# ac-93/tactile_gym

Measured on AMD Instinct MI355X. Metric: env-steps/sec (128x128 tactile obs) at N envs, higher is better.
Workload: dtype f64

## Files before the change

### tactile_gym_amd/csrc/tg_api.hip

```cpp
#include "tg_ctx.hpp"

namespace tg {

int report_error(int code, const char* msg) { return fail(code, msg ? msg : ""); }
static void h_quat_from_euler(const double* rpy, double* q) {
    const double phi = 0.5 * rpy[0], the = 0.5 * rpy[1], psi = 0.5 * rpy[2];
    q[0] = sin(phi) * cos(the) * cos(psi) - cos(phi) * sin(the) * sin(psi);
    q[1] = cos(phi) * sin(the) * cos(psi) + sin(phi) * cos(the) * sin(psi);
    q[2] = cos(phi) * cos(the) * sin(psi) - sin(phi) * sin(the) * cos(psi);
    q[3] = cos(phi) * cos(the) * cos(psi) + sin(phi) * sin(the) * sin(psi);
    const double nrm = sqrt(q[0] * q[0] + q[1] * q[1] + q[2] * q[2] + q[3] * q[3]);
    for (int k = 0; k < 4; ++k) q[k] /= nrm;
}
static void h_mat_from_quat(const double* q, double* R) {
    const double x = q[0], y = q[1], z = q[2], w = q[3];
    const double d = x * x + y * y + z * z + w * w, s = 2.0 / d;
    const double xs = x * s, ys = y * s, zs = z * s, wx = w * xs, wy = w * ys, wz = w * zs, xx = x * xs, xy = x * ys, xz = x * zs, yy = y * ys,
                 yz = y * zs, zz = z * zs;
    R[0] = 1.0 - (yy + zz); R[1] = xy - wz; R[2] = xz + wy;
    R[3] = xy + wz; R[4] = 1.0 - (xx + zz); R[5] = yz - wx;
    R[6] = xz - wy; R[7] = yz + wx; R[8] = 1.0 - (xx + yy);
}


// ... 227 lines not shown
        __syncthreads();
    }
    if (threadIdx.x == 0 && hi[0] > lo[0] && lo[0] != ~0ull) { acc[0] += hi[0] - lo[0]; acc[1] += 1ull; }
}

struct Timer {
    tg_ctx* c; int which; hipEvent_t a = nullptr, b = nullptr;
    Timer(tg_ctx* ctx, int w) : c(ctx), which(w) {
        if ((c->profile || c->profile_clock) && c->d_kt && which < 5) { c->st.kt = c->d_kt; c->rp.kt = c->d_kt; }
        if (c->profile) { (void)hipEventCreate(&a); (void)hipEventCreate(&b); (void)hipEventRecord(a, c->stream); }
    }
    ~Timer() {
        if (c->profile) { (void)hipEventRecord(b, c->stream); c->events.push_back({a, b, which}); }
        if ((c->profile || c->profile_clock) && c->d_kt && which < 5) {
            hipLaunchKernelGGL(k_kt_reduce, dim3(1), dim3(1024), 0, c->stream, c->d_kt, c->kt_slots, c->d_kt_acc + 2 * which);
            c->st.kt = nullptr; c->rp.kt = nullptr;
        }
    }
};


template <typename T, int TOPO> static bool launch_step_t(tg_ctx* c, const float* d_actions, int reset_phase = -1) {
    const int n = c->cfg.num_envs;
    if (c->cfg.control_mode == TG_CONTROL_TCP_POSITION) {
        hipLaunchKernelGGL((k_step_pos<T, TOPO>), dim3((n + 63) / 64), dim3(64), 0, c->stream, (const DevRobot<T>*)c->d_robot,
                           (const EnvConst<T>*)c->d_const, c->st, d_actions);
        return false;
    }
    if constexpr (TOPO == 0 && std::is_same<T, double>::value) {
        if (reset_phase >= 0) {
            hipLaunchKernelGGL((k_step<T, TOPO, true>), dim3((n + 63) / 64), dim3(64), 0, c->stream, (const DevRobot<T>*)c->d_robot,
                               (const EnvConst<T>*)c->d_const, c->st, d_actions, reset_phase, c->bank_mode != 0 ? (const BankDev*)c->d_bank : (const BankDev*)nullptr);
            return true;
        }
    }
    hipLaunchKernelGGL((k_step<T, TOPO>), dim3((n + 63) / 64), dim3(64), 0, c->stream, (const DevRobot<T>*)c->d_robot,
                       (const EnvConst<T>*)c->d_const, c->st, d_actions, -1, (const BankDev*)nullptr);
    return false;
}
template <typename T, int TOPO> static void launch_reset_t(tg_ctx* c, const uint8_t* d_mask, int phase, bool bank = false) {
    const int n = c->cfg.num_envs;
    hipLaunchKernelGGL((k_reset<T, TOPO>), dim3((n + 63) / 64), dim3(64), 0, c->stream, (const DevRobot<T>*)c->d_robot,
                       (const EnvConst<T>*)c->d_const, c->st, d_mask, phase, bank ? (const BankDev*)c->d_bank : (const BankDev*)nullptr);
    if (c->st.kt) c->st.kt += 2 * (size_t)((n + 63) / 64);
}
template <typename T, int TOPO> static void launch_bank_refill_t(tg_ctx* c, int phase) {
    const int n = c->cfg.num_envs;
    hipLaunchKernelGGL((k_bank_refill<T, TOPO>), dim3((n + 63) / 64), dim3(64), 0, c->bank_stream, (const DevRobot<T>*)c->d_robot,
                       (const EnvConst<T>*)c->d_const, c->st, c->bk, c->aux, phase);
}

template <typename T> static void launch_step_body_t(tg_ctx* c, const float* d_actions) {
// ... 587 lines not shown
    if (has_feature) {
        c->packed_feature_off = (c->packed_bytes + 3) & ~(size_t)3;
        c->packed_bytes = c->packed_feature_off + (size_t)n * 12 * 4;
    }
    TG_HIP(hipMalloc(&c->d_obs, c->packed_bytes)); TG_HIP(hipMemset(c->d_obs, 0, c->packed_bytes));
    s.reward = (float*)(c->d_obs + c->packed_obs_bytes);
    s.done = c->d_obs + c->packed_obs_bytes + (size_t)n * 4;
    if (has_feature) s.feature = (float*)(c->d_obs + c->packed_feature_off);
    TG_HIP(hipMalloc(&c->d_term, npix * n)); TG_HIP(hipMemset(c->d_term, 0, npix * n));
    TG_HIP(hipMalloc(&c->d_episode, (size_t)n * 16)); TG_HIP(hipMemset(c->d_episode, 0, (size_t)n * 16));
    s.ep_return = (double*)c->d_episode;
    s.ep_final_return = (float*)(c->d_episode + (size_t)n * 8);
    s.ep_final_len = (int32_t*)(c->d_episode + (size_t)n * 12);
    TG_HIP(hipMalloc(&c->d_mask, n));
#ifdef TG_TL_STAMPS
    TG_HIP(hipMalloc(&s.tl, (4 * 8192 + 4) * 8)); TG_HIP(hipMemset(s.tl, 0, (4 * 8192 + 4) * 8));
#endif
    TG_HIP(hipMalloc(&c->d_actions, (size_t)n * 6 * sizeof(float)));
    c->rp = make_raster_params(W, H, sensor->fov_deg, sensor->near_plane, sensor->far_plane, sensor->turn_off_border, sensor->nodef_dep);
    if (make_block_tables(c->rp, sensor->nodef_dep, sensor->nodef_gray, sensor->border_mask, n, &c->d_block_tables)) return fail(-2, "hipMalloc failed (raster block tables)");
    c->fused_pref = cfg->fused_step == TG_FUSED_OFF ? -1 : cfg->fused_step == TG_FUSED_ON ? 1 : 0;
    if (const char* e = getenv("TG_FUSED_STEP")) c->fused_pref = e[0] == '0' ? -1 : 1;
    c->no_inline_reset = getenv("TG_NO_INLINE_RESET") != nullptr;
#ifdef TG_TL_STAMPS
    c->rp.tl = s.tl;
#endif
    c->bk = s;
    {
        int want = cfg->reset_bank == TG_BANK_OFF ? 0 : cfg->reset_bank == TG_BANK_SYNC ? 2 : 1;
        if (const char* e = getenv("TG_RESET_BANK")) want = (e[0] == '0') ? 0 : (e[0] == 's') ? 2 : 1;
        if (const char* e = getenv("TG_RESET_BANK_EVERY")) { const int k = atoi(e); if (k >= 1) c->bank_every = k; }
        const bool kind_ok = cfg->env_kind == TG_ENV_EDGE_FOLLOW || cfg->env_kind == TG_ENV_SURFACE_FOLLOW_AUTO;
        if (want && kind_ok && cfg->auto_reset && !use_arm_wave(c)) {
            State& b = c->bk;
            auto grab = [&](auto*& ptr, size_t bytes) -> int {
                void* p_ = nullptr;
                if (hipMalloc(&p_, bytes) != hipSuccess) return -1;
                (void)hipMemset(p_, 0, bytes);
                c->bank_allocs.push_back(p_);
                ptr = reinterpret_cast<std::remove_reference_t<decltype(ptr)>>(p_);
                return 0;
            };
            int bad = 0;
            bad |= grab(b.q, nd * 8); bad |= grab(b.qd, nd * 8); bad |= grab(b.qd_target, nd * 8);
            bad |= grab(b.tcp_pos, (size_t)3 * n * 8); bad |= grab(b.tcp_rpy, (size_t)3 * n * 8);
            bad |= grab(b.edge_ang, (size_t)n * 8); bad |= grab(b.embed, (size_t)n * 8); bad |= grab(b.edge_sc, (size_t)2 * n * 8);
// ... 598 lines not shown
```

### tactile_gym_amd/csrc/tg_api_state.hip

```cpp
#include "tg_ctx.hpp"

namespace tg {
template <typename T, int TOPO> static void launch_refresh_t(tg_ctx* c) {
    const int n = c->cfg.num_envs;
    hipLaunchKernelGGL((k_refresh<T, TOPO>), dim3((n + 63) / 64), dim3(64), 0, c->stream, (const DevRobot<T>*)c->d_robot,
                       (const EnvConst<T>*)c->d_const, c->st);
}

template <typename T, int TOPO> static void launch_refresh_rpy_t(tg_ctx* c) {
    const int n = c->cfg.num_envs;
    hipLaunchKernelGGL((k_refresh_rpy<T, TOPO>), dim3((n + 63) / 64), dim3(64), 0, c->stream, (const DevRobot<T>*)c->d_robot,
                       (const EnvConst<T>*)c->d_const, c->st);
}
__global__ __launch_bounds__(256) void k_gather_live_surface(int n, int cells, const uint8_t* __restrict__ hsel, const double* __restrict__ heights,
                                                             const float* __restrict__ zoff, double* __restrict__ out_h, float* __restrict__ out_z) {
    const int env = blockIdx.x;
    const size_t idx = (size_t)(hsel[env] & 3) * n + env;
    if (out_h != nullptr) for (int k = threadIdx.x; k < cells; k += 256) out_h[(size_t)env * cells + k] = heights[idx * cells + k];
    if (out_z != nullptr && threadIdx.x == 0) out_z[env] = zoff[idx];
}
__global__ __launch_bounds__(256) void k_pack_done_rows(const uint8_t* __restrict__ done, const uint8_t* __restrict__ term, const float* __restrict__ ep_ret,
                                                        const int32_t* __restrict__ ep_len, int n, int cap, size_t img, uint8_t* __restrict__ dst) {
    __shared__ int part[256];
    const int env = blockIdx.x, t = threadIdx.x;
// ... 84 lines not shown
    if (!c) return fail(-1, "NULL argument");
    if (!c->d_bp) return fail(-1, "tg_check_broadphase: no guard (tg_set_broadphase)");
    TG_ENTER(c);
    if (launch_broadphase(c->cfg.physics_dtype, c->robot.topology, c->cfg.num_envs, c->stream, c->d_robot, c->d_bp, c->st, c->d_bp_out, c->d_bp_tot))
        return fail(-3, "tg_check_broadphase: unsupported topology");
    TG_HIP(hipGetLastError());
    return 0;
}
int tg_get_broadphase_totals(tg_ctx* c, int64_t* checks, int64_t* pairs, int64_t* hits) {
    if (!c || !checks || !pairs || !hits) return fail(-1, "NULL argument");
    *checks = *pairs = *hits = 0;
    if (!c->d_bp_tot) return 0;
    TG_ENTER(c);
    unsigned long long t[3];
    TG_HIP(hipMemcpyAsync(t, c->d_bp_tot, sizeof t, hipMemcpyDeviceToHost, c->stream));
    TG_HIP(hipStreamSynchronize(c->stream));
    *checks = (int64_t)t[0]; *pairs = (int64_t)t[1]; *hits = (int64_t)t[2];
    return 0;
}

int tg_get_step_mode(tg_ctx* c, int32_t* mode, int32_t* envs_per_wavefront) {
    if (!c || !mode) return fail(-1, "NULL argument");
    *mode = use_fused_step(c) ? 1 : 0;
    if (envs_per_wavefront) *envs_per_wavefront = *mode ? fused_envs_per_wave(c->cfg.num_envs) : 0;
    return 0;
}

int tg_get_actions(tg_ctx* c, void** dev_actions) {
    if (!c || !dev_actions) return fail(-1, "NULL argument");
    *dev_actions = c->d_actions;
    return 0;
}

int tg_get_interior_count(tg_ctx* c, int32_t* k) {
    if (!c || !k) return fail(-1, "NULL argument");
    *k = c->cfg_turn_off_border ? -1 : 4 * c->n_interior;
    return 0;
}
int tg_get_bank_stats(tg_ctx* c, int64_t* swapped, int64_t* late, int32_t* mode) {
    if (!c || !swapped || !late || !mode) return fail(-1, "NULL argument");
    TG_ENTER(c);
    *swapped = 0; *late = 0; *mode = c->bank_mode;
    if (c->st.tmpl_stats != nullptr) {
        unsigned long long t[2] = {0, 0};
        TG_HIP(hipMemcpyAsync(t, c->st.tmpl_stats, 16, hipMemcpyDeviceToHost, c->stream));
        TG_HIP(hipStreamSynchronize(c->stream));
        *swapped = (int64_t)t[0]; *late = (int64_t)t[1]; *mode = c->st.reset_tmpl != nullptr ? 3 : 0;
// ... 177 lines not shown
```

### tactile_gym_amd/csrc/tg_ctx.hpp

```cpp
#pragma once
#include <hip/hip_runtime.h>

#include <chrono>
#include <cmath>
#include <cstdio>
#include <cstdlib>
#include <cstring>
#include <algorithm>
#include <map>
#include <string>
#include <tuple>
#include <type_traits>
#include <vector>

#include "../../include/tactile_gym_hip.h"
#include "tg_kernels.hpp"
#include "tg_contact_wave.h"
#include "tg_spin.h"
#include "tg_fused.h"
#include "tg_scene.h"
#include "tg_noise.h"
#include "tg_raster.h"
#include "tg_exchange.h"
#include "tg_broadphase.h"
// ... 197 lines not shown
    uint64_t random_seed = 0;
    tg::State bk{};
    tg::BankAux aux{};
    int bank_mode = 0;
    uint8_t* h_rows = nullptr;
    size_t h_rows_bytes = 0;
    int bank_every = 8;
    static constexpr int kBankRing = 16, kBankLag = 8;
    hipEvent_t ev_bank_ring[kBankRing] = {};
    unsigned long long bank_visits = 0;
    long long bank_steps = 0;
    hipStream_t bank_stream = nullptr;
    hipEvent_t ev_bank = nullptr, ev_bank_done = nullptr;
    std::vector<void*> bank_allocs;
    void* d_bank = nullptr;
    bool profile = false;
    bool profile_clock = false;
    struct Ev { hipEvent_t a, b; int which; };
    std::vector<Ev> events;
    double prof_ms[6] = {0, 0, 0, 0, 0, 0};
    int64_t prof_n[6] = {0, 0, 0, 0, 0, 0};
    int fused_pref = 0;
    bool no_inline_reset = false;
    unsigned long long* d_kt = nullptr;
    unsigned long long* d_kt_acc = nullptr;
    size_t kt_slots = 0;
    double wall_clock_khz = 100000.0;
};

static inline bool env_has_feature(int env_kind) {
    return env_kind == TG_ENV_OBJECT_PUSH || env_kind == TG_ENV_OBJECT_ROLL || env_kind == TG_ENV_SURFACE_FOLLOW_AUTO;
}

namespace tg {
static void drain_events(tg_ctx* c) {
    for (auto& e : c->events) {
        (void)hipEventSynchronize(e.b);
        float ms = 0;
        (void)hipEventElapsedTime(&ms, e.a, e.b);
        c->prof_ms[e.which] += ms;
        c->prof_n[e.which] += 1;
        (void)hipEventDestroy(e.a); (void)hipEventDestroy(e.b);
    }
    c->events.clear();
}
#define TG_DISPATCH(ctx_dtype, ctx_topo, CALL)                                               \
// ... 54 lines not shown
```

### tactile_gym_amd/csrc/tg_kernels.hpp

```cpp
#pragma once
#include <hip/hip_runtime.h>

#include <stdint.h>

#include "../../include/tactile_gym_hip.h"
#include "tg_physics.hpp"
#include "tg_kt.hpp"

namespace tg {

template <typename T> struct EnvConst {
    int num_envs, act_dim, movement_mode, noise_mode, reward_mode, max_steps, action_repeat, solver_iters;
    T dt, min_action, max_action, act_lo[6], act_hi[6], tcp_lims[6][2];
    T work_pos[3];
    Q4<T> work_q, work_qinv;
    M3<T> work_R, work_Rinv;
    T work_inv_pos[3];
    T stim_pos[3], edge_height, edge_len, term_dist, embed_default;
    double embed_lo, embed_hi;
    M3<T> cam_rot;
    T cam_pos[3];
    int env_kind, surf_rows, surf_cols, surf_goal, surf_vertical;
    M3<T> stim_R;
    double surf_scale, surf_range, surf_interp, surf_extent, auto_scale;
// ... 115 lines not shown
        const double edge = (k == n - 1) ? hi : prod + lo;
        count += (k < n && edge <= v) ? 1 : 0;
    }
    return count;
}
__device__ inline double linspace_value(double lo, double hi, int n, int k) {
#pragma clang fp contract(off)
    const double step = (hi - lo) / (double)(n - 1);
    const double prod = (double)k * step;
    return (k == n - 1) ? hi : prod + lo;
}
__device__ inline double grad_axis(const double* f, int idx, int n, int stride, double h) {
    if (idx == 0) return (f[stride] - f[0]) / h;
    if (idx == n - 1) return (f[(size_t)(n - 1) * stride] - f[(size_t)(n - 2) * stride]) / h;
    return (f[(size_t)(idx + 1) * stride] - f[(size_t)(idx - 1) * stride]) / (2.0 * h);
}

#ifdef TG_KSTEP_STAMPS
__device__ unsigned long long g_kstep_stamps[16];
#define TG_KSTAMP(i) { if (blockIdx.x == 0 && threadIdx.x == 0) g_kstep_stamps[i] = __builtin_readcyclecounter(); asm volatile("" ::: "memory"); }
#else
#define TG_KSTAMP(i)
#endif
__device__ __forceinline__ void episode_step(const State& st, int env, float reward, bool done, int step_count) {
    const double acc = st.ep_return[env] + (double)reward;
    if (done) { st.ep_final_return[env] = (float)acc; st.ep_final_len[env] = step_count; }
    st.ep_return[env] = done ? 0.0 : acc;
}

template <typename T, int TOPO>
__device__ __forceinline__ bool finish_env(const DevRobot<T>& m, const EnvConst<T>& c, const State& st, int env, const T (&q)[Topo<TOPO>::N],
                                           T edge_ang, int step_count, bool write_reward_done, const JointTrig<T, Topo<TOPO>::N>* trig = nullptr,
                                           bool lazy_rpy = false ) {
    const int n = c.num_envs;
    bool done_flag = false;
    Kin<T, TOPO> k;
    if (trig != nullptr) forward_kinematics<T, TOPO, true>(m, q, k, trig);
    else forward_kinematics<T, TOPO>(m, q, k);
    V3<T> ptcp; M3<T> Rtcp;
    link_frame<T, TOPO>(k, m.tcp_link, m.tcp_pos, m.tcp_rot, ptcp, Rtcp);
    st.tcp_pos[0 * n + env] = (double)ptcp.x; st.tcp_pos[1 * n + env] = (double)ptcp.y; st.tcp_pos[2 * n + env] = (double)ptcp.z;
    if (!lazy_rpy) {
        T rpy[3];
        { Q4<T> qq = quat_from_mat(Rtcp); euler_from_quat(qq, rpy[0], rpy[1], rpy[2]); }
        st.tcp_rpy[0 * n + env] = (double)rpy[0]; st.tcp_rpy[1 * n + env] = (double)rpy[1]; st.tcp_rpy[2 * n + env] = (double)rpy[2];
    }
    T se = T(0), ce = T(1);
    if (c.env_kind == TG_ENV_EDGE_FOLLOW) {
        if (lazy_rpy) { se = (T)st.edge_sc[0 * n + env]; ce = (T)st.edge_sc[1 * n + env]; }
        else { tsincos(edge_ang, &se, &ce); st.edge_sc[0 * n + env] = (double)se; st.edge_sc[1 * n + env] = (double)ce; }
    }
    if (write_reward_done && c.env_kind == TG_ENV_EDGE_FOLLOW) {
        const T gx = c.stim_pos[0] + c.edge_len * ce, gy = c.stim_pos[1] + c.edge_len * se;
        const T dx = ptcp.x - gx, dy = ptcp.y - gy;
        const T goal_dist = tsqrt(dx * dx + dy * dy);
        const bool done = goal_dist < c.term_dist || step_count >= c.max_steps;
        const T p1x = c.stim_pos[0] - c.edge_len * ce, p1y = c.stim_pos[1] - c.edge_len * se;
        const T d21x = gx - p1x, d21y = gy - p1y, d13x = p1x - ptcp.x, d13y = p1y - ptcp.y;
        const T edge_dist = tabs(d21x * d13y - d21y * d13x) / tsqrt(d21x * d21x + d21y * d21y);
        T reward;
        if (c.reward_mode == TG_REWARD_SPARSE) reward = goal_dist < c.term_dist ? T(1) : T(0);
        else reward = -((T(1) * goal_dist) + (T(10) * edge_dist) + T(0));
        st.reward[env] = (float)reward;
        st.done[env] = done ? 1 : 0;
        done_flag = done;
        episode_step(st, env, (float)reward, done, step_count);
    }
    TG_KSTAMP(5)
    if ((write_reward_done || c.reward_mode == TG_REWARD_SPARSE) && c.env_kind == TG_ENV_SURFACE_FOLLOW_AUTO) {
        const int R = c.surf_rows, Cc = c.surf_cols;
        int ti = digitize_linspace((double)ptcp.y, c.ybin_lo, c.ybin_hi, Cc);
        int tj = digitize_linspace((double)ptcp.x, c.xbin_lo, c.xbin_hi, R);
        if (ti == Cc) ti -= 1;
        if (tj == R) tj -= 1;
        const double* H = st.heights + ((size_t)(st.hsel[env] & 3) * n + env) * R * Cc;
        const T surf_z = (T)(H[(size_t)ti * Cc + tj] + (double)c.stim_pos[2]);
        const T gy_ = (T)grad_axis(H + tj, ti, R, Cc, c.surf_scale);
        const T gx_ = (T)grad_axis(H + (size_t)ti * Cc, tj, Cc, 1, c.surf_scale);
        V3<T> nrm{-gx_, -gy_, T(1)};
        nrm = (T(1) / norm(nrm)) * nrm;
        const T gdx = ptcp.x - (T)st.goal[0 * n + env], gdy = ptcp.y - (T)st.goal[1 * n + env], gdz = ptcp.z - (T)st.goal[2 * n + env];
        T reward;
        if (c.surf_vertical) {
            nrm = mul(c.stim_R, nrm);
            const V3<T> tipv = mul(Rtcp, mk(T(-1), T(0), T(0)));
            const V3<T> emb = mul(Rtcp, mk(-c.embed_default, T(0), T(0)));
            const T surf_x = (T)((double)c.stim_pos[0] - H[(size_t)ti * Cc + tj]);
            const T surf_dist = tabs((ptcp.x + emb.x) - surf_x);
            const T cos_sim = dot(nrm, tipv) / (norm(nrm) * norm(tipv));
            reward = -((T(10) * surf_dist) + (T(3) * (T(1) - cos_sim)));
        } else {
            const V3<T> tipv = mul(Rtcp, mk(T(0), T(0), T(-1)));
            const V3<T> emb = mul(Rtcp, mk(T(0), T(0), -c.embed_default));
            const T surf_dist = tabs((ptcp.z + emb.z) - surf_z);
            const T cos_sim = dot(nrm, tipv) / (norm(nrm) * norm(tipv));
            const T w_norm = (c.movement_mode == TG_SMOVE_YZ || c.movement_mode == TG_SMOVE_XYZ) ? T(0) : T(1);
            reward = c.surf_goal ? -((T(1) * tsqrt(gdx * gdx + gdy * gdy)) + (T(10) * surf_dist) + (w_norm * (T(1) - cos_sim)))
                                 : -((T(1) * surf_dist) + (w_norm * (T(1) - cos_sim)));
        }
        const bool at_goal = tsqrt(gdx * gdx + gdy * gdy + gdz * gdz) < c.term_dist;
        T out = reward;
        if (c.reward_mode == TG_REWARD_SPARSE) {
            const double acc = st.accum[env] + (double)reward;
            st.accum[env] = acc;
            out = at_goal ? (T)acc : T(0);
        }
        if (write_reward_done) {
            st.reward[env] = (float)out;
            st.done[env] = (at_goal || step_count >= c.max_steps) ? 1 : 0;
            done_flag = at_goal || step_count >= c.max_steps;
            episode_step(st, env, (float)out, at_goal || step_count >= c.max_steps, step_count);
        }
    }
    if (c.env_kind == TG_ENV_SURFACE_FOLLOW_AUTO && st.feature != nullptr) {
        const V3<T> tw_ = load_v3(c.work_inv_pos) + mul(c.work_Rinv, ptcp);
        const V3<T> gw_ = load_v3(c.work_inv_pos) + mul(c.work_Rinv, mk((T)st.goal[0 * n + env], (T)st.goal[1 * n + env], (T)st.goal[2 * n + env]));
        const float f[6] = {(float)tw_.x, (float)tw_.y, (float)tw_.z, (float)gw_.x, (float)gw_.y, (float)gw_.z};
#pragma unroll
        for (int e = 0; e < 6; ++e) {
            st.feature[(size_t)env * 12 + e] = f[e];
            if (write_reward_done) st.term_feature[(size_t)env * 12 + e] = f[e];
        }
    }
    TG_KSTAMP(6)
    V3<T> pb; M3<T> Rb;
    link_frame<T, TOPO>(k, m.sensor_link, m.sensor_pos, m.sensor_rot, pb, Rb);
    const V3<T> pc = pb + mul(Rb, load_v3(c.cam_pos));
    const M3<T> Rc = mul(Rb, c.cam_rot);
    V3<T> f{Rc.m[0], Rc.m[3], Rc.m[6]}, up{Rc.m[2], Rc.m[5], Rc.m[8]};
    f = (T(1) / norm(f)) * f;
    V3<T> s = cross(f, up);
    s = (T(1) / norm(s)) * s;
    const V3<T> u = cross(s, f);
    V3<T> ox{ce, se, T(0)}, oy{-se, ce, T(0)}, oz{T(0), T(0), T(1)};
    if (c.surf_vertical) {
        ox = mk(c.stim_R.m[0], c.stim_R.m[3], c.stim_R.m[6]); oy = mk(c.stim_R.m[1], c.stim_R.m[4], c.stim_R.m[7]);
        oz = mk(c.stim_R.m[2], c.stim_R.m[5], c.stim_R.m[8]);
    }
    const V3<T> dp = load_v3(c.stim_pos) - pc;
    const V3<T> nf = mk<T>(0, 0, 0) - f;
    float* X = st.stim_xform;
    X[0 * n + env] = (float)dot(s, ox);  X[1 * n + env] = (float)dot(s, oy);  X[2 * n + env] = (float)dot(s, oz);
    X[3 * n + env] = (float)dot(u, ox);  X[4 * n + env] = (float)dot(u, oy);  X[5 * n + env] = (float)dot(u, oz);
    X[6 * n + env] = (float)dot(nf, ox); X[7 * n + env] = (float)dot(nf, oy); X[8 * n + env] = (float)dot(nf, oz);
    X[9 * n + env] = (float)dot(s, dp);  X[10 * n + env] = (float)dot(u, dp); X[11 * n + env] = (float)dot(nf, dp);
    return done_flag;
}

template <typename T, int TOPO>
__global__ __launch_bounds__(64) void k_oracle_obs(const DevRobot<T>* __restrict__ mp, const EnvConst<T>* __restrict__ cp, State st, int dim,
                                                   float* __restrict__ out) {
    constexpr int N = Topo<TOPO>::N;
// ... 158 lines not shown
            for (int r = 0; r < 3; ++r) g[r] = (double)c.work_pos[r] + ((double)c.work_R.m[3 * r + 0] * wx + (double)c.work_R.m[3 * r + 1] * wy);
            put_sphere(i, g, 0.01f, i < gid ? 255.0f : 0.0f, i > gid ? 255.0f : 0.0f, i == gid ? 255.0f : 0.0f);
        }
    } else if (c.env_kind == TG_ENV_OBJECT_ROLL) {
        const M3<T> Rq = mat_from_quat(quat_from_mat(Rtcp));
        const V3<T> gw = ptcp + mul(Rq, mk((T)st.goal[0 * n + env], (T)st.goal[1 * n + env], (T)st.goal[2 * n + env]));
        const double g[3] = {(double)gw.x, (double)gw.y, (double)gw.z};
        put_sphere(0, g, 0.0025f, 255.0f, 0.0f, 0.0f);
    } else {
        for (int i = 0; i < n_spheres; ++i) S[8 * i + 7] = 0.0f;
    }
}

template <typename T> __device__ __forceinline__ void scale_actions(const EnvConst<T>& c, const T (&enc)[6], T (&vels)[6]) {
    const T in_range = c.max_action - c.min_action;
#pragma unroll
    for (int d = 0; d < 6; ++d) {
        T x = enc[d];
        x = x < c.min_action ? c.min_action : (x > c.max_action ? c.max_action : x);
        vels[d] = (((x - c.min_action) * (c.act_hi[d] - c.act_lo[d])) / in_range) + c.act_lo[d];
    }
}

template <typename T, int TOPO>
__device__ __forceinline__ void tcp_velocity_control(const DevRobot<T>& m, const EnvConst<T>& c, const T (&q)[Topo<TOPO>::N], T (&vels)[6],
                                                     T (&qd_des)[Topo<TOPO>::N], const JointTrig<T, Topo<TOPO>::N>* trig = nullptr,
                                                     T work_dz = T(0) ) {
    constexpr int N = Topo<TOPO>::N;
    Kin<T, TOPO> k;
    if (trig != nullptr) forward_kinematics<T, TOPO, true>(m, q, k, trig);
    else forward_kinematics<T, TOPO>(m, q, k);
    V3<T> ptcp; M3<T> Rtcp;
    link_frame<T, TOPO>(k, m.tcp_link, m.tcp_pos, m.tcp_rot, ptcp, Rtcp);
    TG_KSTAMP(10)
    V3<T> wpos; T wrpy[3] = {T(0), T(0), T(0)}, rpyw[3];
    if (__any(vels[3] != T(0) || vels[4] != T(0) || vels[5] != T(0)))
        world_to_work<T, false>(c, mk(ptcp.x, ptcp.y, ptcp.z - work_dz), Rtcp, wpos, wrpy, rpyw);
    else
        wpos = load_v3(c.work_inv_pos) + mul(c.work_Rinv, mk(ptcp.x, ptcp.y, ptcp.z - work_dz));
    const T cur[6] = {wpos.x, wpos.y, wpos.z, wrpy[0], wrpy[1], wrpy[2]};
#pragma unroll
    for (int d = 0; d < 6; ++d) {
        const bool ex = (cur[d] < c.tcp_lims[d][0] && vels[d] < T(0)) || (cur[d] > c.tcp_lims[d][1] && vels[d] > T(0));
        if (ex) vels[d] = T(0);
    }
    const V3<T> lin = mul(c.work_R, mk(vels[0], vels[1], vels[2]));
    const V3<T> ang = mul(c.work_R, mk(vels[3], vels[4], vels[5]));
    TG_KSTAMP(11)
    T J[6][N];
    tcp_jacobian<T, TOPO>(m, k, ptcp, J);
    TG_KSTAMP(12)
    if (N == 6) {
        T A[6][6], b[6] = {lin.x, lin.y, lin.z, ang.x, ang.y, ang.z}, x[6];
#pragma unroll
        for (int r = 0; r < 6; ++r)
#pragma unroll
            for (int cc = 0; cc < 6; ++cc) A[r][cc] = J[r][cc < N ? cc : 0];
        solve_pivoted<T, 6>(A, b, x);
#pragma unroll
        for (int i = 0; i < N; ++i) qd_des[i] = x[i < 6 ? i : 0];
    } else {
        const T b[6] = {lin.x, lin.y, lin.z, ang.x, ang.y, ang.z};
        pinv_apply<T, N>(J, b, qd_des);
        if (N == 8) { qd_des[N - 3] = qd_des[1]; qd_des[N - 2] = -qd_des[1]; qd_des[N - 1] = qd_des[1] + qd_des[2]; }
    }
}

template <typename T>
__device__ __forceinline__ void encode_arm_actions(const EnvConst<T>& c, const State& st, int env, const float* __restrict__ a, T (&enc)[6]) {
    const int n = c.num_envs;
    if (c.env_kind == TG_ENV_EDGE_FOLLOW) {
        enc[0] = (T)a[0]; enc[1] = (T)a[1];
        if (c.movement_mode == TG_MOVE_XYZ) enc[2] = (T)a[2];
        else if (c.movement_mode == TG_MOVE_XYRZ) enc[5] = (T)a[2];
        else if (c.movement_mode == TG_MOVE_XYZRZ) { enc[2] = (T)a[2]; enc[5] = (T)a[3]; }
    } else if (c.surf_goal) {
        if (c.movement_mode == TG_SMOVE_YZ) { enc[1] = (T)a[0]; enc[2] = (T)a[1]; }
        else if (c.movement_mode == TG_SMOVE_YZRX) { enc[1] = (T)a[0]; enc[2] = (T)a[1]; enc[3] = (T)a[2]; }
        else {
            enc[0] = (T)a[0]; enc[1] = (T)a[1]; enc[2] = (T)a[2];
            if (c.movement_mode == TG_SMOVE_XYZRXRY) { enc[3] = (T)a[3]; enc[4] = (T)a[4]; }
        }
    } else if (c.surf_vertical) {
        enc[1] = (T)((st.dir[1 * n + env] * (double)c.max_action) * c.auto_scale);
        enc[0] = (T)a[0]; enc[5] = (T)a[1];
    } else {
        enc[0] = (T)((st.dir[0 * n + env] * (double)c.max_action) * c.auto_scale);
        enc[1] = (T)((st.dir[1 * n + env] * (double)c.max_action) * c.auto_scale);
        enc[2] = (T)a[0];
        if (c.movement_mode == TG_SMOVE_YZRX) enc[3] = (T)a[1];
        else if (c.movement_mode == TG_SMOVE_XYZRXRY) { enc[3] = (T)a[1]; enc[4] = (T)a[2]; }
    }
}

template <typename T, int TOPO>
__device__ __forceinline__ bool step_env(const DevRobot<T>& m, const EnvConst<T>& c, const State& st, int env, const float* __restrict__ actions,
                                         bool* done_out = nullptr ) {
    constexpr int N = Topo<TOPO>::N;
    const int n = c.num_envs;
    TG_KSTAMP(0)
    T q[N], qd[N];
#pragma unroll
    for (int i = 0; i < N; ++i) { q[i] = (T)st.q[i * n + env]; qd[i] = (T)st.qd[i * n + env]; }
    T enc[6] = {T(0), T(0), T(0), T(0), T(0), T(0)};
    if (st.draw != nullptr) {
        const uint64_t counter = st.draw[0] + 1, seed = st.draw[1];
        const float lo = (float)c.min_action, hi = (float)c.max_action;
        float abuf[6] = {0.0f, 0.0f, 0.0f, 0.0f, 0.0f, 0.0f};
#pragma unroll
        for (int j = 0; j < 6; ++j) {
            if (j < c.act_dim) {
                const int i = env * c.act_dim + j;
                const uint64_t z = mix64(mix64(seed + kGolden * (counter + 1)) + kGolden * (uint64_t)(i + 1));
                const float u = (float)(uint32_t)(z >> 40) * (1.0f / 16777216.0f);
                abuf[j] = lo + (hi - lo) * u;
                st.act_out[i] = abuf[j];
            }
        }
        encode_arm_actions<T>(c, st, env, abuf, enc);
    } else {
        encode_arm_actions<T>(c, st, env, actions + (size_t)env * c.act_dim, enc);
    }
    T vels[6];
    scale_actions<T>(c, enc, vels);
    const int step_count = st.step_count[env] + 1;
    st.step_count[env] = step_count;
    JointTrig<T, N> trig;
    const int lic = st.licence[env];
    if (__all(lic > 0)) {
#pragma unroll
        for (int i = 0; i < N; ++i) { trig.s[i] = (T)st.trig_sc[i * n + env]; trig.c[i] = (T)st.trig_sc[(8 + i) * n + env]; }
    } else {
        trig_init<T, N>(q, trig);
    }
    T qd_des[N];
    TG_KSTAMP(1)
    tcp_velocity_control<T, TOPO>(m, c, q, vels, qd_des, &trig);
    TG_KSTAMP(2)
#pragma unroll
    for (int i = 0; i < N; ++i) st.qd_target[i * n + env] = (double)qd_des[i];

    T qdummy[N];
#pragma unroll
    for (int i = 0; i < N; ++i) qdummy[i] = T(0);
    int verified = __all(lic > 0) ? 24 : 0;
    bool ran_full = false;
    int sweeps = 0;
    for (int t = 0; t < c.action_repeat; ++t) {
        const int before = verified;
        sim_tick<T, TOPO, kMotorVelocity, true, true>(m, q, qd, qdummy, qd_des, T(0), m.vel_gain, m.max_force, c.dt, c.solver_iters, &trig,
                                                      &verified, &sweeps);
        const bool analytic = before > 0 && verified == before - 1;
        if (t == 0) TG_KSTAMP(7)
        if (!analytic) ran_full = true;
        if (verified < 0) verified = 0;
        const int remaining = c.action_repeat - t - 1;
        if (analytic && remaining > 0 && verified >= remaining && c.solver_iters >= 0) {
            T v2 = T(0);
#pragma unroll
            for (int i = 0; i < N; ++i) v2 += qd[i] * qd[i];
// ... 4 lines not shown
                for (int i = 0; i < N; ++i) dq[i] = c.dt * qd[i];
                for (int r = 0; r < remaining; ++r) {
#pragma unroll
                    for (int i = 0; i < N; ++i) q[i] += dq[i];
                }
                T dqt[N];
#pragma unroll
                for (int i = 0; i < N; ++i) dqt[i] = (T)remaining * dq[i];
                trig_advance<T, N>(q, dqt, trig);
                verified -= remaining;
                break;
            }
        }
    }
    st.licence[env] = ran_full ? (verified > 0 ? 8 : 0) : lic - 1;
    if (m.res_thr > T(0)) st.sweeps[env] = sweeps;
    TG_KSTAMP(3)

#pragma unroll
    for (int i = 0; i < N; ++i) { st.q[i * n + env] = (double)q[i]; st.qd[i * n + env] = (double)qd[i]; }
#pragma unroll
    for (int i = 0; i < N; ++i) { st.trig_sc[i * n + env] = (double)trig.s[i]; st.trig_sc[(8 + i) * n + env] = (double)trig.c[i]; }
    TG_KSTAMP(4)
    const bool done = finish_env<T, TOPO>(m, c, st, env, q, (T)st.edge_ang[env], step_count, true, &trig, true);
    if (done_out != nullptr) *done_out = done;
    return ran_full;
}
constexpr int kDrawGroups = 32, kDrawWords = 16 + 16 * kDrawGroups;
__device__ __forceinline__ void draw_counter_advance(const State& st) {
    if (st.draw != nullptr) {
        __syncthreads();
        if (threadIdx.x == 0) {
            bool last = true;
            if (gridDim.x > 2 * kDrawGroups) {
                const unsigned g = blockIdx.x % kDrawGroups;
                const unsigned long long members = (gridDim.x - g + kDrawGroups - 1) / kDrawGroups;
                unsigned long long* tk = st.draw + 16 + 16 * g;
                last = atomicAdd(tk, 1ull) == members - 1;
                if (last) { atomicExch(tk, 0ull); last = atomicAdd(st.draw + 2, 1ull) == (unsigned long long)kDrawGroups - 1; }
            } else {
                last = atomicAdd(st.draw + 2, 1ull) == (unsigned long long)gridDim.x - 1;
            }
            if (last) { atomicExch(st.draw + 2, 0ull); atomicAdd(st.draw + 0, 1ull); }
        }
    }
}

// ... 7 lines not shown
        const unsigned g = blockIdx.x % kDrawGroups;
        const unsigned long long members = (gridDim.x - g + kDrawGroups - 1) / kDrawGroups;
        last = ticket == members - 1;
        if (last) { atomicExch(st.draw + 16 + 16 * g, 0ull); last = atomicAdd(st.draw + 2, 1ull) == (unsigned long long)kDrawGroups - 1; }
    } else {
        last = ticket == (unsigned long long)gridDim.x - 1;
    }
    if (last) { atomicExch(st.draw + 2, 0ull); atomicAdd(st.draw + 0, 1ull); }
}

template <typename T, int TOPO> __device__ __forceinline__ void reset_or_swap(const DevRobot<T>* __restrict__ mp, const EnvConst<T>* __restrict__ cp, const State& st,
                                                                             int env, bool in_step, int phase, const BankDev* __restrict__ bd);
template <typename T, int TOPO, bool RESET = false>
__global__ __launch_bounds__(64) void k_step(const DevRobot<T>* __restrict__ mp, const EnvConst<T>* __restrict__ cp, State st,
                                             const float* __restrict__ actions, int reset_phase, const BankDev* __restrict__ bd) {
    KtScope kt_scope_(st.kt);
    const int env = blockIdx.x * blockDim.x + threadIdx.x;
    TG_TL(st.tl, 1);
    if (env >= cp->num_envs) return;
    bool done = false;
    const bool ran_full = step_env<T, TOPO>(*mp, *cp, st, env, actions, &done);
    if (RESET) {
        if (done) reset_or_swap<T, TOPO>(mp, cp, st, env, true, reset_phase, bd);
    }
    draw_counter_advance(st);
    TG_KSTAMP(9)
#ifdef TG_KSTEP_STAMPS
    if (blockIdx.x == 0 && threadIdx.x == 0) g_kstep_stamps[15] = ran_full ? 1 : 0;
#else
    (void)ran_full;
#endif
}

template <typename T> __device__ __forceinline__ V3<T> rot_error(const M3<T>& Rt, const M3<T>& R) {
    M3<T> E;
#pragma unroll
    for (int i = 0; i < 3; ++i)
#pragma unroll
        for (int j = 0; j < 3; ++j) E.m[3 * i + j] = Rt.m[3 * i] * R.m[3 * j] + Rt.m[3 * i + 1] * R.m[3 * j + 1] + Rt.m[3 * i + 2] * R.m[3 * j + 2];
    const T cosang = T(0.5) * (E.m[0] + E.m[4] + E.m[8] - T(1));
    const V3<T> ax{E.m[7] - E.m[5], E.m[2] - E.m[6], E.m[3] - E.m[1]};
    const T s = norm(ax);
    const T ang = tatan2(T(0.5) * s, cosang);
    if (s < T(1e-12)) return T(0.5) * ax;
    return (ang / s) * ax;
}
// ... 1330 lines not shown
```

### tactile_gym_amd/csrc/tg_physics.hpp

```cpp
#pragma once
#include <hip/hip_runtime.h>
#include <stdint.h>

#include <type_traits>

namespace tg {

constexpr int kMaxDof = 8;
constexpr int kMaxBodiesPerLink = 4;

template <int TOPO> struct Topo;
template <> struct Topo<0> {
    static constexpr int N = 6;
    static constexpr int NP = 6;
    __host__ __device__ static constexpr int parent(int i) { return i - 1; }
};
template <> struct Topo<1> {
    static constexpr int N = 8;
    static constexpr int NP = 5;
    __host__ __device__ static constexpr int parent(int i) { return i == 0 ? -1 : (i == 5 ? 0 : i - 1); }
};
template <int TOPO> __host__ __device__ constexpr bool is_ancestor_or_self(int anc, int i) {
    while (i >= 0) { if (i == anc) return true; i = Topo<TOPO>::parent(i); }
    return false;
// ... 169 lines not shown
        if (p < 0) {
            k.R[i] = Rl;
            k.o[i] = load_v3(m.jpos[i]);
        } else {
            k.R[i] = mul(k.R[p], Rl);
            k.o[i] = k.o[p] + mul(k.R[p], load_v3(m.jpos[i]));
        }
        k.a[i] = mul(k.R[i], ax);
    }
}

template <typename T, int TOPO> __device__ __forceinline__ void link_frame(const Kin<T, TOPO>& k, int link, const T* fpos, const T* frot,
                                                                             V3<T>& pos, M3<T>& rot) {
    constexpr int N = Topo<TOPO>::N;
#pragma unroll
    for (int i = 0; i < N; ++i) {
        if (i == link) {
            pos = k.o[i] + mul(k.R[i], load_v3(fpos));
            rot = mul(k.R[i], load_m3(frot));
        }
    }
}

template <typename T, int TOPO, bool BIAS = true, bool TRIG = false>
__device__ __forceinline__ void dynamics_terms(const DevRobot<T>& m, const T (&q)[Topo<TOPO>::N], const T (&qd)[Topo<TOPO>::N],
                                               T (&hbias)[Topo<TOPO>::N], T (&qdamp)[Topo<TOPO>::N],
                                               T (&Minv)[Topo<TOPO>::N][Topo<TOPO>::N], T& traceM, const V3<T> g, Kin<T, TOPO>& k,
                                               const JointTrig<T, Topo<TOPO>::N>* trig = nullptr) {
    constexpr int N = Topo<TOPO>::N;
    forward_kinematics<T, TOPO, TRIG>(m, q, k, trig);
    V3<T> w[N], wd[N], vo[N], ao[N];
    V3<T> WF[N], WN[N], DF[N], DN[N], hc[N];
    S3<T> Io[N];
    T mc[N];
#pragma unroll
    for (int i = 0; i < N; ++i) {
        const int p = Topo<TOPO>::parent(i);
        const V3<T> aq = qd[i] * k.a[i];
        if (p < 0) {
            w[i] = aq;
            vo[i] = mk<T>(0, 0, 0);
            if (BIAS) {
                wd[i] = mk<T>(0, 0, 0);
                ao[i] = mk<T>(0, 0, 0) - g;
            }
        } else {
// ... 1556 lines not shown
```

Measured before the change: 27.43 million.

## Add quad-lane step kernel splitting forward kinematics rows across four lanes

Adds k_step_quad, enabled by default for TOPO 0 with double precision. It assigns four lanes to each environment. Forward kinematics is computed row-wise, one rotation row per lane, and the rows are reassembled with DPP quad broadcasts. Per-env state reads are preloaded so that the redundant lanes do not read values another lane has already overwritten, and only lane 0 performs resets. The aim is to shorten the serial per-env critical path and register pressure in the step kernel, at the cost of four times as many threads doing mostly redundant work elsewhere and duplicate identical stores. Action encoding is also made branchless.

```diff
diff --git a/tactile_gym_amd/csrc/tg_api.hip b/tactile_gym_amd/csrc/tg_api.hip
--- a/tactile_gym_amd/csrc/tg_api.hip
+++ b/tactile_gym_amd/csrc/tg_api.hip
@@ -273,12 +273,24 @@
 
 template <typename T, int TOPO> static bool launch_step_t(tg_ctx* c, const float* d_actions, int reset_phase = -1) {
     const int n = c->cfg.num_envs;
+    c->step_envs_per_wave = 64;
     if (c->cfg.control_mode == TG_CONTROL_TCP_POSITION) {
         hipLaunchKernelGGL((k_step_pos<T, TOPO>), dim3((n + 63) / 64), dim3(64), 0, c->stream, (const DevRobot<T>*)c->d_robot,
                            (const EnvConst<T>*)c->d_const, c->st, d_actions);
         return false;
     }
     if constexpr (TOPO == 0 && std::is_same<T, double>::value) {
+        if (c->kstep_quad) {
+            const dim3 grid((unsigned)((4 * (size_t)n + 63) / 64));
+            c->step_envs_per_wave = 16;
+            if (reset_phase >= 0)
+                hipLaunchKernelGGL((k_step_quad<T, true>), grid, dim3(64), 0, c->stream, (const DevRobot<T>*)c->d_robot, (const EnvConst<T>*)c->d_const,
+                                   c->st, d_actions, reset_phase, c->bank_mode != 0 ? (const BankDev*)c->d_bank : (const BankDev*)nullptr);
+            else
+                hipLaunchKernelGGL((k_step_quad<T, false>), grid, dim3(64), 0, c->stream, (const DevRobot<T>*)c->d_robot, (const EnvConst<T>*)c->d_const,
+                                   c->st, d_actions, -1, (const BankDev*)nullptr);
+            return reset_phase >= 0;
+        }
         if (reset_phase >= 0) {
             hipLaunchKernelGGL((k_step<T, TOPO, true>), dim3((n + 63) / 64), dim3(64), 0, c->stream, (const DevRobot<T>*)c->d_robot,
                                (const EnvConst<T>*)c->d_const, c->st, d_actions, reset_phase, c->bank_mode != 0 ? (const BankDev*)c->d_bank : (const BankDev*)nullptr);
@@ -912,6 +924,7 @@
     c->fused_pref = cfg->fused_step == TG_FUSED_OFF ? -1 : cfg->fused_step == TG_FUSED_ON ? 1 : 0;
     if (const char* e = getenv("TG_FUSED_STEP")) c->fused_pref = e[0] == '0' ? -1 : 1;
     c->no_inline_reset = getenv("TG_NO_INLINE_RESET") != nullptr;
+    { const char* e = getenv("TG_KSTEP_QUAD"); c->kstep_quad = !(e != nullptr && e[0] == '0'); }
 #ifdef TG_TL_STAMPS
     c->rp.tl = s.tl;
 #endif
diff --git a/tactile_gym_amd/csrc/tg_api_state.hip b/tactile_gym_amd/csrc/tg_api_state.hip
--- a/tactile_gym_amd/csrc/tg_api_state.hip
+++ b/tactile_gym_amd/csrc/tg_api_state.hip
@@ -130,7 +130,7 @@
 int tg_get_step_mode(tg_ctx* c, int32_t* mode, int32_t* envs_per_wavefront) {
     if (!c || !mode) return fail(-1, "NULL argument");
     *mode = use_fused_step(c) ? 1 : 0;
-    if (envs_per_wavefront) *envs_per_wavefront = *mode ? fused_envs_per_wave(c->cfg.num_envs) : 0;
+    if (envs_per_wavefront) *envs_per_wavefront = *mode ? fused_envs_per_wave(c->cfg.num_envs) : c->step_envs_per_wave;
     return 0;
 }
 
diff --git a/tactile_gym_amd/csrc/tg_ctx.hpp b/tactile_gym_amd/csrc/tg_ctx.hpp
--- a/tactile_gym_amd/csrc/tg_ctx.hpp
+++ b/tactile_gym_amd/csrc/tg_ctx.hpp
@@ -243,6 +243,8 @@
     int64_t prof_n[6] = {0, 0, 0, 0, 0, 0};
     int fused_pref = 0;
     bool no_inline_reset = false;
+    int step_envs_per_wave = 0;
+    bool kstep_quad = true;
     unsigned long long* d_kt = nullptr;
     unsigned long long* d_kt_acc = nullptr;
     size_t kt_slots = 0;
diff --git a/tactile_gym_amd/csrc/tg_kernels.hpp b/tactile_gym_amd/csrc/tg_kernels.hpp
--- a/tactile_gym_amd/csrc/tg_kernels.hpp
+++ b/tactile_gym_amd/csrc/tg_kernels.hpp
@@ -161,32 +161,51 @@
 #else
 #define TG_KSTAMP(i)
 #endif
-__device__ __forceinline__ void episode_step(const State& st, int env, float reward, bool done, int step_count) {
-    const double acc = st.ep_return[env] + (double)reward;
+__device__ __forceinline__ void episode_step(const State& st, int env, float reward, bool done, int step_count,
+                                             const double* prev = nullptr ) {
+    const double acc = (prev != nullptr ? *prev : st.ep_return[env]) + (double)reward;
     if (done) { st.ep_final_return[env] = (float)acc; st.ep_final_len[env] = step_count; }
     st.ep_return[env] = done ? 0.0 : acc;
 }
 
+template <typename T, typename TcpRot, typename CamFrame>
+__device__ __forceinline__ bool finish_env_from(const EnvConst<T>& c, const State& st, int env, V3<T> ptcp, TcpRot rot, CamFrame cam, T edge_ang,
+                                                int step_count, bool write_reward_done, bool lazy_rpy, const T* pre_sc = nullptr,
+                                                const double* pre_ep = nullptr);
 template <typename T, int TOPO>
 __device__ __forceinline__ bool finish_env(const DevRobot<T>& m, const EnvConst<T>& c, const State& st, int env, const T (&q)[Topo<TOPO>::N],
                                            T edge_ang, int step_count, bool write_reward_done, const JointTrig<T, Topo<TOPO>::N>* trig = nullptr,
                                            bool lazy_rpy = false ) {
-    const int n = c.num_envs;
-    bool done_flag = false;
     Kin<T, TOPO> k;
     if (trig != nullptr) forward_kinematics<T, TOPO, true>(m, q, k, trig);
     else forward_kinematics<T, TOPO>(m, q, k);
     V3<T> ptcp; M3<T> Rtcp;
     link_frame<T, TOPO>(k, m.tcp_link, m.tcp_pos, m.tcp_rot, ptcp, Rtcp);
+    return finish_env_from<T>(c, st, env, ptcp, [&]() { return Rtcp; },
+                              [&](V3<T>& pc, V3<T>& f, V3<T>& up) {
+                                  V3<T> pb; M3<T> Rb;
+                                  link_frame<T, TOPO>(k, m.sensor_link, m.sensor_pos, m.sensor_rot, pb, Rb);
+                                  pc = pb + mul(Rb, load_v3(c.cam_pos));
+                                  const M3<T> Rc = mul(Rb, c.cam_rot);
+                                  f = mk(Rc.m[0], Rc.m[3], Rc.m[6]); up = mk(Rc.m[2], Rc.m[5], Rc.m[8]);
+                              },
+                              edge_ang, step_count, write_reward_done, lazy_rpy);
+}
+template <typename T, typename TcpRot, typename CamFrame>
+__device__ __forceinline__ bool finish_env_from(const EnvConst<T>& c, const State& st, int env, V3<T> ptcp, TcpRot rot, CamFrame cam, T edge_ang,
+                                                int step_count, bool write_reward_done, bool lazy_rpy, const T* pre_sc, const double* pre_ep) {
+    const int n = c.num_envs;
+    bool done_flag = false;
     st.tcp_pos[0 * n + env] = (double)ptcp.x; st.tcp_pos[1 * n + env] = (double)ptcp.y; st.tcp_pos[2 * n + env] = (double)ptcp.z;
     if (!lazy_rpy) {
         T rpy[3];
-        { Q4<T> qq = quat_from_mat(Rtcp); euler_from_quat(qq, rpy[0], rpy[1], rpy[2]); }
+        { Q4<T> qq = quat_from_mat(rot()); euler_from_quat(qq, rpy[0], rpy[1], rpy[2]); }
         st.tcp_rpy[0 * n + env] = (double)rpy[0]; st.tcp_rpy[1 * n + env] = (double)rpy[1]; st.tcp_rpy[2 * n + env] = (double)rpy[2];
     }
     T se = T(0), ce = T(1);
     if (c.env_kind == TG_ENV_EDGE_FOLLOW) {
-        if (lazy_rpy) { se = (T)st.edge_sc[0 * n + env]; ce = (T)st.edge_sc[1 * n + env]; }
+        if (lazy_rpy && pre_sc != nullptr) { se = pre_sc[0]; ce = pre_sc[1]; }
+        else if (lazy_rpy) { se = (T)st.edge_sc[0 * n + env]; ce = (T)st.edge_sc[1 * n + env]; }
         else { tsincos(edge_ang, &se, &ce); st.edge_sc[0 * n + env] = (double)se; st.edge_sc[1 * n + env] = (double)ce; }
     }
     if (write_reward_done && c.env_kind == TG_ENV_EDGE_FOLLOW) {
@@ -203,7 +222,7 @@
         st.reward[env] = (float)reward;
         st.done[env] = done ? 1 : 0;
         done_flag = done;
-        episode_step(st, env, (float)reward, done, step_count);
+        episode_step(st, env, (float)reward, done, step_count, pre_ep);
     }
     TG_KSTAMP(5)
     if ((write_reward_done || c.reward_mode == TG_REWARD_SPARSE) && c.env_kind == TG_ENV_SURFACE_FOLLOW_AUTO) {
@@ -219,6 +238,7 @@
         V3<T> nrm{-gx_, -gy_, T(1)};
         nrm = (T(1) / norm(nrm)) * nrm;
         const T gdx = ptcp.x - (T)st.goal[0 * n + env], gdy = ptcp.y - (T)st.goal[1 * n + env], gdz = ptcp.z - (T)st.goal[2 * n + env];
+        const M3<T> Rtcp = rot();
         T reward;
         if (c.surf_vertical) {
             nrm = mul(c.stim_R, nrm);
@@ -248,7 +268,7 @@
             st.reward[env] = (float)out;
             st.done[env] = (at_goal || step_count >= c.max_steps) ? 1 : 0;
             done_flag = at_goal || step_count >= c.max_steps;
-            episode_step(st, env, (float)out, at_goal || step_count >= c.max_steps, step_count);
+            episode_step(st, env, (float)out, at_goal || step_count >= c.max_steps, step_count, pre_ep);
         }
     }
     if (c.env_kind == TG_ENV_SURFACE_FOLLOW_AUTO && st.feature != nullptr) {
@@ -262,11 +282,8 @@
         }
     }
     TG_KSTAMP(6)
-    V3<T> pb; M3<T> Rb;
-    link_frame<T, TOPO>(k, m.sensor_link, m.sensor_pos, m.sensor_rot, pb, Rb);
-    const V3<T> pc = pb + mul(Rb, load_v3(c.cam_pos));
-    const M3<T> Rc = mul(Rb, c.cam_rot);
-    V3<T> f{Rc.m[0], Rc.m[3], Rc.m[6]}, up{Rc.m[2], Rc.m[5], Rc.m[8]};
+    V3<T> pc, f, up;
+    cam(pc, f, up);
     f = (T(1) / norm(f)) * f;
     V3<T> s = cross(f, up);
     s = (T(1) / norm(s)) * s;
@@ -471,20 +488,28 @@
     }
 }
 
+template <typename T, int TOPO, typename TcpRot>
+__device__ __forceinline__ void tcp_velocity_solve(const DevRobot<T>& m, const EnvConst<T>& c, const Kin<T, TOPO>& k, V3<T> ptcp, TcpRot rot,
+                                                   T (&vels)[6], T (&qd_des)[Topo<TOPO>::N], T work_dz);
 template <typename T, int TOPO>
 __device__ __forceinline__ void tcp_velocity_control(const DevRobot<T>& m, const EnvConst<T>& c, const T (&q)[Topo<TOPO>::N], T (&vels)[6],
                                                      T (&qd_des)[Topo<TOPO>::N], const JointTrig<T, Topo<TOPO>::N>* trig = nullptr,
                                                      T work_dz = T(0) ) {
-    constexpr int N = Topo<TOPO>::N;
     Kin<T, TOPO> k;
     if (trig != nullptr) forward_kinematics<T, TOPO, true>(m, q, k, trig);
     else forward_kinematics<T, TOPO>(m, q, k);
     V3<T> ptcp; M3<T> Rtcp;
     link_frame<T, TOPO>(k, m.tcp_link, m.tcp_pos, m.tcp_rot, ptcp, Rtcp);
     TG_KSTAMP(10)
+    tcp_velocity_solve<T, TOPO>(m, c, k, ptcp, [&]() { return Rtcp; }, vels, qd_des, work_dz);
+}
+template <typename T, int TOPO, typename TcpRot>
+__device__ __forceinline__ void tcp_velocity_solve(const DevRobot<T>& m, const EnvConst<T>& c, const Kin<T, TOPO>& k, V3<T> ptcp, TcpRot rot,
+                                                   T (&vels)[6], T (&qd_des)[Topo<TOPO>::N], T work_dz) {
+    constexpr int N = Topo<TOPO>::N;
     V3<T> wpos; T wrpy[3] = {T(0), T(0), T(0)}, rpyw[3];
     if (__any(vels[3] != T(0) || vels[4] != T(0) || vels[5] != T(0)))
-        world_to_work<T, false>(c, mk(ptcp.x, ptcp.y, ptcp.z - work_dz), Rtcp, wpos, wrpy, rpyw);
+        world_to_work<T, false>(c, mk(ptcp.x, ptcp.y, ptcp.z - work_dz), rot(), wpos, wrpy, rpyw);
     else
         wpos = load_v3(c.work_inv_pos) + mul(c.work_Rinv, mk(ptcp.x, ptcp.y, ptcp.z - work_dz));
     const T cur[6] = {wpos.x, wpos.y, wpos.z, wrpy[0], wrpy[1], wrpy[2]};
@@ -515,14 +540,49 @@
     }
 }
 
+template <typename T, int TOPO>
+__device__ __forceinline__ void tcp_velocity_control_quad(const DevRobot<T>& m, const EnvConst<T>& c, T (&vels)[6], T (&qd_des)[Topo<TOPO>::N],
+                                                          const JointTrig<T, Topo<TOPO>::N>& trig) {
+    constexpr int N = Topo<TOPO>::N;
+    KinRow<T, TOPO> kr;
+    forward_kinematics_quad<T, TOPO>(m, kr, trig);
+    T pr; V3<T> Rr;
+    link_frame_quad<T, TOPO>(kr, m.tcp_link, m.tcp_pos, m.tcp_rot, pr, Rr);
+    const V3<T> ptcp = quad_gather(pr);
+    Kin<T, TOPO> k;
+#pragma unroll
+    for (int i = 0; i < N; ++i) { k.o[i] = quad_gather(kr.o[i]); k.a[i] = quad_gather(kr.a[i]); }
+    TG_KSTAMP(10)
+    tcp_velocity_solve<T, TOPO>(m, c, k, ptcp, [&]() { return quad_gather(Rr); }, vels, qd_des, T(0));
+}
+template <typename T, int TOPO>
+__device__ __forceinline__ bool finish_env_quad(const DevRobot<T>& m, const EnvConst<T>& c, const State& st, int env, T edge_ang, int step_count,
+                                                const JointTrig<T, Topo<TOPO>::N>& trig, const T (&pre_sc)[2], const double& pre_ep) {
+    KinRow<T, TOPO> kr;
+    forward_kinematics_quad<T, TOPO>(m, kr, trig);
+    T pr; V3<T> Rr;
+    link_frame_quad<T, TOPO>(kr, m.tcp_link, m.tcp_pos, m.tcp_rot, pr, Rr);
+    return finish_env_from<T>(c, st, env, quad_gather(pr), [&]() { return quad_gather(Rr); },
+                              [&](V3<T>& pc, V3<T>& f, V3<T>& up) {
+                                  T pbr; V3<T> Rbr;
+                                  link_frame_quad<T, TOPO>(kr, m.sensor_link, m.sensor_pos, m.sensor_rot, pbr, Rbr);
+                                  const T pcr = pbr + row_dot(Rbr, load_v3(c.cam_pos));
+                                  const V3<T> Rcr = row_mul(Rbr, c.cam_rot);
+                                  pc = quad_gather(pcr); f = quad_gather(Rcr.x); up = quad_gather(Rcr.z);
+                              },
+                              edge_ang, step_count, true, true, pre_sc, &pre_ep);
+}
+
 template <typename T>
 __device__ __forceinline__ void encode_arm_actions(const EnvConst<T>& c, const State& st, int env, const float* __restrict__ a, T (&enc)[6]) {
     const int n = c.num_envs;
     if (c.env_kind == TG_ENV_EDGE_FOLLOW) {
         enc[0] = (T)a[0]; enc[1] = (T)a[1];
-        if (c.movement_mode == TG_MOVE_XYZ) enc[2] = (T)a[2];
-        else if (c.movement_mode == TG_MOVE_XYRZ) enc[5] = (T)a[2];
-        else if (c.movement_mode == TG_MOVE_XYZRZ) { enc[2] = (T)a[2]; enc[5] = (T)a[3]; }
+        const int mm = c.movement_mode;
+        const T a2 = (mm == TG_MOVE_XYZ || mm == TG_MOVE_XYRZ || mm == TG_MOVE_XYZRZ) ? (T)a[2] : T(0);
+        const T a3 = (mm == TG_MOVE_XYZRZ) ? (T)a[3] : T(0);
+        enc[2] = (mm == TG_MOVE_XYZ || mm == TG_MOVE_XYZRZ) ? a2 : enc[2];
+        enc[5] = mm == TG_MOVE_XYRZ ? a2 : (mm == TG_MOVE_XYZRZ ? a3 : enc[5]);
     } else if (c.surf_goal) {
         if (c.movement_mode == TG_SMOVE_YZ) { enc[1] = (T)a[0]; enc[2] = (T)a[1]; }
         else if (c.movement_mode == TG_SMOVE_YZRX) { enc[1] = (T)a[0]; enc[2] = (T)a[1]; enc[3] = (T)a[2]; }
@@ -542,7 +602,7 @@
     }
 }
 
-template <typename T, int TOPO>
+template <typename T, int TOPO, bool QUAD = false>
 __device__ __forceinline__ bool step_env(const DevRobot<T>& m, const EnvConst<T>& c, const State& st, int env, const float* __restrict__ actions,
                                          bool* done_out = nullptr ) {
     constexpr int N = Topo<TOPO>::N;
@@ -551,6 +611,15 @@
     T q[N], qd[N];
 #pragma unroll
     for (int i = 0; i < N; ++i) { q[i] = (T)st.q[i * n + env]; qd[i] = (T)st.qd[i * n + env]; }
+    int pre_lic = 0, pre_count = 0;
+    T pre_ts[N], pre_tc[N], pre_sc[2] = {T(0), T(1)};
+    double pre_ep = 0.0;
+    if constexpr (QUAD) {
+        pre_lic = st.licence[env]; pre_count = st.step_count[env]; pre_ep = st.ep_return[env];
+#pragma unroll
+        for (int i = 0; i < N; ++i) { pre_ts[i] = (T)st.trig_sc[i * n + env]; pre_tc[i] = (T)st.trig_sc[(8 + i) * n + env]; }
+        if (c.env_kind == TG_ENV_EDGE_FOLLOW) { pre_sc[0] = (T)st.edge_sc[0 * n + env]; pre_sc[1] = (T)st.edge_sc[1 * n + env]; }
+    }
     T enc[6] = {T(0), T(0), T(0), T(0), T(0), T(0)};
     if (st.draw != nullptr) {
         const uint64_t counter = st.draw[0] + 1, seed = st.draw[1];
@@ -572,19 +641,23 @@
     }
     T vels[6];
     scale_actions<T>(c, enc, vels);
-    const int step_count = st.step_count[env] + 1;
+    const int step_count = (QUAD ? pre_count : st.step_count[env]) + 1;
     st.step_count[env] = step_count;
     JointTrig<T, N> trig;
-    const int lic = st.licence[env];
+    const int lic = QUAD ? pre_lic : st.licence[env];
     if (__all(lic > 0)) {
 #pragma unroll
-        for (int i = 0; i < N; ++i) { trig.s[i] = (T)st.trig_sc[i * n + env]; trig.c[i] = (T)st.trig_sc[(8 + i) * n + env]; }
+        for (int i = 0; i < N; ++i) {
+            if constexpr (QUAD) { trig.s[i] = pre_ts[i]; trig.c[i] = pre_tc[i]; }
+            else { trig.s[i] = (T)st.trig_sc[i * n + env]; trig.c[i] = (T)st.trig_sc[(8 + i) * n + env]; }
+        }
     } else {
         trig_init<T, N>(q, trig);
     }
     T qd_des[N];
     TG_KSTAMP(1)
-    tcp_velocity_control<T, TOPO>(m, c, q, vels, qd_des, &trig);
+    if constexpr (QUAD) tcp_velocity_control_quad<T, TOPO>(m, c, vels, qd_des, trig);
+    else tcp_velocity_control<T, TOPO>(m, c, q, vels, qd_des, &trig);
     TG_KSTAMP(2)
 #pragma unroll
     for (int i = 0; i < N; ++i) st.qd_target[i * n + env] = (double)qd_des[i];
@@ -635,7 +708,9 @@
 #pragma unroll
     for (int i = 0; i < N; ++i) { st.trig_sc[i * n + env] = (double)trig.s[i]; st.trig_sc[(8 + i) * n + env] = (double)trig.c[i]; }
     TG_KSTAMP(4)
-    const bool done = finish_env<T, TOPO>(m, c, st, env, q, (T)st.edge_ang[env], step_count, true, &trig, true);
+    bool done;
+    if constexpr (QUAD) done = finish_env_quad<T, TOPO>(m, c, st, env, T(0) , step_count, trig, pre_sc, pre_ep);
+    else done = finish_env<T, TOPO>(m, c, st, env, q, (T)st.edge_ang[env], step_count, true, &trig, true);
     if (done_out != nullptr) *done_out = done;
     return ran_full;
 }
@@ -689,6 +764,27 @@
     const bool ran_full = step_env<T, TOPO>(*mp, *cp, st, env, actions, &done);
     if (RESET) {
         if (done) reset_or_swap<T, TOPO>(mp, cp, st, env, true, reset_phase, bd);
+    }
+    draw_counter_advance(st);
+    TG_KSTAMP(9)
+#ifdef TG_KSTEP_STAMPS
+    if (blockIdx.x == 0 && threadIdx.x == 0) g_kstep_stamps[15] = ran_full ? 1 : 0;
+#else
+    (void)ran_full;
+#endif
+}
+
+template <typename T, bool RESET = false>
+__global__ __launch_bounds__(64) void k_step_quad(const DevRobot<T>* __restrict__ mp, const EnvConst<T>* __restrict__ cp, State st,
+                                                  const float* __restrict__ actions, int reset_phase, const BankDev* __restrict__ bd) {
+    KtScope kt_scope_(st.kt);
+    const int env = (int)((blockIdx.x * blockDim.x + threadIdx.x) >> 2);
+    TG_TL(st.tl, 1);
+    if (env >= cp->num_envs) return;
+    bool done = false;
+    const bool ran_full = step_env<T, 0, true>(*mp, *cp, st, env, actions, &done);
+    if (RESET) {
+        if (done && (threadIdx.x & 3) == 0) reset_or_swap<T, 0>(mp, cp, st, env, true, reset_phase, bd);
     }
     draw_counter_advance(st);
     TG_KSTAMP(9)
diff --git a/tactile_gym_amd/csrc/tg_physics.hpp b/tactile_gym_amd/csrc/tg_physics.hpp
--- a/tactile_gym_amd/csrc/tg_physics.hpp
+++ b/tactile_gym_amd/csrc/tg_physics.hpp
@@ -215,6 +215,66 @@
     }
 }
 
+template <typename T, int TOPO> struct KinRow {
+    static constexpr int N = Topo<TOPO>::N;
+    V3<T> R[N];
+    T o[N], a[N];
+};
+__device__ __forceinline__ int quad_row() { const int r = (int)(threadIdx.x & 3); return r == 3 ? 2 : r; }
+template <typename T> __device__ __forceinline__ T pick3(int r, T x, T y, T z) { return r == 0 ? x : (r == 1 ? y : z); }
+template <typename T> __device__ __forceinline__ V3<T> row_mul(V3<T> a, const M3<T>& B) {
+    return {a.x * B.m[0] + a.y * B.m[3] + a.z * B.m[6], a.x * B.m[1] + a.y * B.m[4] + a.z * B.m[7], a.x * B.m[2] + a.y * B.m[5] + a.z * B.m[8]};
+}
+template <typename T> __device__ __forceinline__ T row_dot(V3<T> a, V3<T> v) { return a.x * v.x + a.y * v.y + a.z * v.z; }
+template <int K> __device__ __forceinline__ double quad_bcast(double x) {
+    const long long b = __double_as_longlong(x);
+    const int lo = __builtin_amdgcn_update_dpp(0, (int)(b & 0xffffffffll), K * 0x55, 0xF, 0xF, false);
+    const int hi = __builtin_amdgcn_update_dpp(0, (int)(b >> 32), K * 0x55, 0xF, 0xF, false);
+    return __longlong_as_double(((long long)hi << 32) | (long long)(unsigned)lo);
+}
+template <int K> __device__ __forceinline__ float quad_bcast(float x) {
+    return __int_as_float(__builtin_amdgcn_update_dpp(0, __float_as_int(x), K * 0x55, 0xF, 0xF, false));
+}
+template <typename T> __device__ __forceinline__ V3<T> quad_gather(T x) { return {quad_bcast<0>(x), quad_bcast<1>(x), quad_bcast<2>(x)}; }
+template <typename T> __device__ __forceinline__ M3<T> quad_gather(V3<T> row) {
+    const V3<T> c0 = quad_gather(row.x), c1 = quad_gather(row.y), c2 = quad_gather(row.z);
+    return M3<T>{{c0.x, c1.x, c2.x, c0.y, c1.y, c2.y, c0.z, c1.z, c2.z}};
+}
+
+template <typename T, int TOPO>
+__device__ __forceinline__ void forward_kinematics_quad(const DevRobot<T>& m, KinRow<T, TOPO>& k, const JointTrig<T, Topo<TOPO>::N>& trig) {
+    constexpr int N = Topo<TOPO>::N;
+    const int r = quad_row();
+#pragma unroll
+    for (int i = 0; i < N; ++i) {
+        const int p = Topo<TOPO>::parent(i);
+        const V3<T> ax = load_v3(m.jaxis[i]);
+        const T sq = trig.s[i], cq = trig.c[i];
+        M3<T> Rl;
+#pragma unroll
+        for (int e = 0; e < 9; ++e) Rl.m[e] = m.fkA[i][e] + cq * m.fkB[i][e] + sq * m.fkC[i][e];
+        if (p < 0) {
+            k.R[i] = mk(pick3(r, Rl.m[0], Rl.m[3], Rl.m[6]), pick3(r, Rl.m[1], Rl.m[4], Rl.m[7]), pick3(r, Rl.m[2], Rl.m[5], Rl.m[8]));
+            k.o[i] = pick3(r, m.jpos[i][0], m.jpos[i][1], m.jpos[i][2]);
+        } else {
+            k.R[i] = row_mul(k.R[p], Rl);
+            k.o[i] = k.o[p] + row_dot(k.R[p], load_v3(m.jpos[i]));
+        }
+        k.a[i] = row_dot(k.R[i], ax);
+    }
+}
+template <typename T, int TOPO> __device__ __forceinline__ void link_frame_quad(const KinRow<T, TOPO>& k, int link, const T* fpos, const T* frot,
+                                                                                  T& pos, V3<T>& rot) {
+    constexpr int N = Topo<TOPO>::N;
+#pragma unroll
+    for (int i = 0; i < N; ++i) {
+        if (i == link) {
+            pos = k.o[i] + row_dot(k.R[i], load_v3(fpos));
+            rot = row_mul(k.R[i], load_m3(frot));
+        }
+    }
+}
+
 template <typename T, int TOPO, bool BIAS = true, bool TRIG = false>
 __device__ __forceinline__ void dynamics_terms(const DevRobot<T>& m, const T (&q)[Topo<TOPO>::N], const T (&qd)[Topo<TOPO>::N],
                                                T (&hbias)[Topo<TOPO>::N], T (&qdamp)[Topo<TOPO>::N],
```

After: 30.29 million, median of 6. +10.4%, better.
